# nathancunn/ParticleMDI.jl

Measured on AMD Instinct MI355X. Metric: Gibbs iters/sec (and obs·particles/sec) at 1/2/4/8 GPUs vs CPU ref, higher is better.
Workload: dtype f64

## Files before the change

### particlemdi.jl_amd/csrc/pmdi_sweep2_body.h

```cpp
#pragma once
#include "pmdi_arith.h"
#include "pmdi_internal.h"

#ifndef PM2_LANE_API_PROVIDED
#define PM2_DEV __device__ __forceinline__
#define PM2_COLD __device__ __noinline__
#define PM2_HD inline __host__ __device__
extern __shared__ __attribute__((aligned(16))) unsigned char pm2_smem_[];
#define PM2_SMEM (pm2_smem_)
#define PM2_TID() ((int)threadIdx.x)
#define PM2_BID() ((int)blockIdx.x)
#define PM2_BALLOT(p) __ballot(p)
#define PM2_SHFL64(v, src) pm2_shfl64((v), (src))
#define PM2_WAVE_BARRIER() do { __builtin_amdgcn_fence(__ATOMIC_ACQ_REL, "wavefront"); __builtin_amdgcn_wave_barrier(); } while (0)
#define PM2_BARRIER() __syncthreads()
#define PM2_LDS_BARRIER() asm volatile("s_waitcnt lgkmcnt(0)\n\ts_barrier" ::: "memory")
#define PM2_UNI(x) __builtin_amdgcn_readfirstlane(x)
#define PM2_CLOCK() ((long long)clock64())
#define PM2_WALLCLOCK() ((long long)wall_clock64())
#if defined(__HIP_DEVICE_COMPILE__)
#define PM2_G(T, p) ((__attribute__((address_space(1))) T *)(p))
#define PM2_CONST __attribute__((address_space(4)))
#ifdef PM2_NO_LAUNDER
#define PM2_LAUNDER(ptr_, T) do { } while (0)
// ... 112 lines not shown
#define PHD(i_) PHXW(15)
#define PHR(i_) do { } while (0)
#define PHC(i_) PHXW(i_)
#else
#define PHD(i_) PHX(i_)
#define PHR(i_) do { } while (0)
#define PHC(i_) do { } while (0)
#endif
#else
#define PHD(i_) do { } while (0)
#define PHR(i_) do { } while (0)
#define PHC(i_) do { } while (0)
#endif

typedef unsigned long long u64;
typedef unsigned short u16;
typedef unsigned char u8;

constexpr int NWMAX = 8;
#ifndef PM2_NS
#define PM2_NS 8
#endif
constexpr int NS = PM2_NS;
constexpr int XR = 4;
#ifndef PM2_XCAP
#define PM2_XCAP 24
#endif
constexpr int XCAP = PM2_XCAP;
constexpr int NR = (NS > 2 * XR) ? NS : 2 * XR;
constexpr int CLSMAX = 32;
PM2_HD constexpr int class_slot_bits(int K, int PPL, int NW) { return (K == 4 && PPL == 4 && NW == 4) ? 4 : 5; }
PM2_HD constexpr int class_slots_max(int K, int PPL, int NW) { return 1 << class_slot_bits(K, PPL, NW); }
PM2_HD constexpr bool cdf_rows_in_arena(int NW) { return NW > 4; }
constexpr int KCAPMAX = 256;
constexpr int RI_CLSMIN = 64, RI_NEWSLOT = 96, RI_CLSVAL = 128;
constexpr int RI_WCNT = 160;
constexpr int RD_MAX = 0, RD_MIN = NWMAX, RD_SA = 2 * NWMAX, RD_SQ = 3 * NWMAX;
constexpr int KMAX2 = 4;
constexpr int NONE8 = 0xFF;
constexpr unsigned INFU = 0xFFFFFFFFu;
constexpr int PMDI_S2_REQUEUE = 1;

enum { DS_MAXID = 0, DS_NCLS, DS_NCOL, DS_NDX, DS_ND, DS_NS0, DS_NX, DS_NNEED, DS_NCLONE, DS_NFLAG, DS_FOLLOW, DS_DIRTY, DS_NEEDMASK, DS_CHANGED, DS_NDLOW, DS_HALT, DS_COUNT = 16 };
enum { SC_FAIL = 0, SC_RES, SC_PSTAR, SC_NLEAF, SC_NPROG, SC_JS, SC_TMP0, SC_TMP1, SC_TMP2, SC_TMP3, SC_COUNT = 16 };

typedef S2Layout Layout;

PM2_HD void make_layout(int K, int N, int P, int Dmax, int cols_l, int idcap, int cls, int cdfl, Layout &L)
{
    const int CLS = cls;
    const int kcap = (CLS * N < KCAPMAX) ? CLS * N : KCAPMAX;
    if (cdfl > cls) cdfl = cls;
    L.cls = cls; L.kcap = kcap; L.cdfl = cdfl;
    int o = 0;
    auto take = [&](int bytes) { const int at = o; o = (o + bytes + 15) & ~15; return at; };
    const int Dp = (Dmax + 1) & ~1;
    L.Dp = Dp; L.cols_l = cols_l; L.idcap = idcap;
    L.red = take(128 * 8);
    L.sc = take(SC_COUNT * 4);
    L.stat = take(8 * 8);
    L.wk = take(KMAX2 * 8 * 8);
    L.ph = take(16 * 8);
    L.leaf_i1 = 0; L.leaf_n = 0; L.leaf_prog = 0;
    L.leaf_tot = take(64 * 8); L.leaf_carry = take(64 * 8);
    L.xfl = take(KMAX2 * 64);
    L.tr_tb = 0;
    L.tr_cdf = 128 * 8;
    L.tr_stride = L.tr_cdf + cdfl * (N + 2) * 8;
    if (L.tr_stride < NR * Dp * 8) L.tr_stride = NR * Dp * 8;
    L.tr_stride = (L.tr_stride + 15) & ~15;
    L.rs_jtab = P * 8; L.rs_raw = P * 10; L.rs_anc = P * 12; L.rs_hist = P * 14;
    const int rs = P * 14 + idcap * 4 + 64;
    int trb = K * L.tr_stride;
    if (trb < rs) trb = rs;
    L.tr_bytes = trb;
    L.tr = take(trb);
    const int b0 = o;
// ... 82 lines not shown
    PM2_DEV double *lp() const { return lds<double>(base + lay->lp); }
    PM2_DEV double lp_get(int j) const { if (j < NS + XCAP) return lp()[j]; return PM2_G(const double, ar.lpx())[j - NS - XCAP]; }
    PM2_DEV void lp_set(int j, double x) const { if (j < NS + XCAP) lp()[j] = x; else PM2_G(double, ar.lpx())[j - NS - XCAP] = x; }
    PM2_DEV int xid_get(int e) const { if (e < XCAP) return lds<int>(base + lay->xid)[e]; return PM2_G(const int, ar.xidx())[e - XCAP]; }
    PM2_DEV void xid_set(int e, int id) const { if (e < XCAP) lds<int>(base + lay->xid)[e] = id; else PM2_G(int, ar.xidx())[e - XCAP] = id; }
};

PM2_DEV int popc_below64(const u64 *bm, int p)
{
    int n = 0;
    const int w = p >> 6;
    for (int i = 0; i < w; ++i) n += pm2_popc64(bm[i]);
    return n + pm2_popc64(bm[w] & ((1ull << (p & 63)) - 1ull));
}

template <class Tp, int NN>
struct RegArr {
    Tp head;
    RegArr<Tp, NN - 1> tail;
    PM2_DEV Tp operator[](int i) const { return i == 0 ? head : tail[i - 1]; }
    PM2_DEV void set(int i, Tp x) { head = (i == 0) ? x : head; tail.set(i - 1, x); }
};
template <class Tp>
struct RegArr<Tp, 1> {
    Tp head;
    PM2_DEV Tp operator[](int) const { return head; }
    PM2_DEV void set(int i, Tp x) { head = (i == 0) ? x : head; }
};

template <class Ds> PM2_DEV int ds_levels(const Ds &d) { return d.L; }

template <int K, int PPL, int NW, bool GO> struct Sweep2;
template <int K, int PPL, int NW, bool GO> PM2_COLD void hand_over_cold(Sweep2<K, PPL, NW, GO> s, long long pos, int fcode, long long t_start);

template <int K, int PPL, int NW, bool GO>
struct Sweep2 {
    static constexpr int T = 64 * NW;
    static_assert(NW >= K && NW <= NWMAX, "one owner wave per dataset");
    RegArr<double, PPL> lw;
    static constexpr int NCP = (PPL + 1) / 2;
    RegArr<unsigned, K * NCP> colp;
    static constexpr bool CDFA = cdf_rows_in_arena(NW);
    PM2_DEV double cdf_get(const DV &v, int r, int j) const { if (!CDFA || r < v.cdfl) return v.cdf_row_l(r)[j]; return PM2_G(const double, v.ar.cdfg())[(size_t)r * (N + 2) + j]; }
    PM2_DEV void cdf_set(const DV &v, int r, int j, double x) const { if (!CDFA || r < v.cdfl) v.cdf_row_l(r)[j] = x; else PM2_G(double, v.ar.cdfg())[(size_t)r * (N + 2) + j] = x; }
    static constexpr int CSB = class_slot_bits(K, PPL, NW);
    static constexpr bool ONEWORD = CSB * K * PPL <= 64;
    static constexpr int NCSW = ONEWORD ? 1 : K;
    template <bool Wide, class Dummy = void> struct CslWord { typedef unsigned type; };
    template <class Dummy> struct CslWord<true, Dummy> { typedef u64 type; };
    typedef typename CslWord<(ONEWORD || CSB * PPL > 32)>::type csl_t;
    RegArr<csl_t, NCSW> cslp;
    static_assert(CSB * PPL <= 64, "class slots of a lane's particles of one dataset must fit one 64-bit word");
    RegArr<double, NS> c_mu, c_lam;
#ifdef PM2_DETAIL_TIMERS
    long long phd_last;
    int phd_cur;
#endif
    double pend_g;
    int pend_slot;
    const PM2_CONST SweepArgs *ap;
    int tid, lane, wave, chain;
    int N, P;
    unsigned long long seed;
    unsigned iter;
    long long n, n1;

// ... 992 lines not shown
        const int nb = P >> 6;
        double *lv = car;
        if (wave == 0) {
            if (tid == 0) lds<double>(L.red)[121] = w[0];
            for (int h = 1; (nb >> h) >= 2; ++h) {
                const int cnt = nb >> h, off = nb - (nb >> (h - 1)), offp = (h >= 2) ? nb - (nb >> (h - 2)) : 0;
                if (lane < cnt) {
                    double val;
                    if (h == 1) val = (lane == 0) ? tot[1] : tot[2 * lane] + tot[2 * lane + 1];
                    else val = lv[offp + 2 * lane] + lv[offp + 2 * lane + 1];
                    lv[off + lane] = val;
                }
                PM2_WAVE_BARRIER();
            }
        }
        PM2_BARRIER();
        double carry = lds<double>(L.red)[121];
        if (blk >= 2) {
            const int j = 32 - __builtin_clz((unsigned)blk);
            carry = carry + lv[nb - (nb >> (j - 2))];
            for (int h = j - 2; h >= 0; --h)
                if ((blk >> h) & 1) {
                    const int g = (blk >> h) - 1;
                    carry = carry + (h == 0 ? tot[g] : lv[nb - (nb >> (h - 1)) + g]);
                }
        }
#pragma unroll
        for (int u = 0; u < PPL; ++u) {
            const int p = tid * PPL + u;
            c[u] = (p == 0) ? w[u] : carry + sl[u];
        }
    }

    PM2_DEV void resample(long long pos, double mx)
    {
        PHR(0);
        double w[PPL];
#pragma unroll
        for (int u = 0; u < PPL; ++u) w[u] = exp(lw[u] - mx);
        const double u01 = pmdi_arith::uniform01(seed, iter, (unsigned)pos, 0, 0, SITE_RESAMPLE_U);
        const double usl = pmdi_arith::uniform01(seed, iter, (unsigned)pos, 0, 0, SITE_RESAMPLE_SLOT);
        double c[PPL];
        PHR(1);
        cumsum_pairwise(w, c);
        PHR(2);
        double *utab = lds<double>(L.tr);
        u16 *jtab = lds<u16>(L.tr + L.rs_jtab), *raw = lds<u16>(L.tr + L.rs_raw), *anc = lds<u16>(L.tr + L.rs_anc);
        double *red = lds<double>(L.red);
        if (tid == T - 1) red[0] = c[PPL - 1];
        {
            const double h = 1.0 / (double)P;
            const int j = tid * PPL;
            double u = u01 / (double)P;
            int done = 0;
            while (done < j) {
                int e;
                (void)frexp(u, &e);
                const double B = ldexp(1.0, e);
                const double xx = (B - u) * (double)P;
                double m = floor(xx);
                if (m == xx) m -= 1.0;
                if (m > (double)(j - done)) m = (double)(j - done);
                if (m >= 1.0) { u = u + m * h; done += (int)m; }
                if (done < j) { u = u + h; done += 1; }
            }
#pragma unroll
// ... 9 lines not shown
                int J = (int)((q - utab[0]) * (double)P) + 1;
                if (J < 0) J = 0;
                if (J > P) J = P;
                while (J < P && q >= utab[J]) ++J;
                while (J > 0 && !(q >= utab[J - 1])) --J;
                jtab[tid * PPL + uu] = (u16)J;
            }
        }
        PM2_BARRIER();
        PHR(4);
        {
            int lo = 0;
#pragma unroll
            for (int uu = 0; uu < PPL; ++uu) {
                const int j = tid * PPL + uu;
                if (uu == 0 || !((int)jtab[lo] > j)) {
                    int hi = P - 1;
                    while (lo < hi) { const int mid = (lo + hi) >> 1; if ((int)jtab[mid] > j) hi = mid; else lo = mid + 1; }
                }
                raw[j] = (u16)lo;
            }
        }
        int js = (int)(usl * (double)P);
        if (js >= P) js = P - 1;
        PM2_BARRIER();
        PHR(5);
#pragma unroll
        for (int uu = 0; uu < PPL; ++uu) {
            const int p = tid * PPL + uu;
            anc[p] = (p == 0) ? (u16)0 : (p <= js ? raw[p - 1] : raw[p]);
            lw.set(uu, 1.0);
        }
        PM2_BARRIER();
        u16 *scol = lds<u16>(L.tr), *mult = lds<u16>(L.tr + P * 2), *cmap = lds<u16>(L.tr + P * 4);
        u8 *scsl = lds<u8>(L.tr + P * 6);
        int *hist = lds<int>(L.tr + L.rs_hist);
#pragma nounroll
        for (int k = 0; k < K; ++k) {
            const DV v = view(k);
            int *dsc = v.dsc();
            const int ncol_old = dsc[DS_NCOL], oldmax = dsc[DS_MAXID], ncls_old = dsc[DS_NCLS];
            PHR(6);
            int ck[PPL], rk[PPL];
            col_get(k, ck);
#pragma unroll
            for (int uu = 0; uu < PPL; ++uu) rk[uu] = csl_get(k, uu);
#pragma unroll
            for (int uu = 0; uu < PPL; ++uu) { const int p = tid * PPL + uu; scol[p] = (u16)ck[uu]; scsl[p] = (u8)rk[uu]; }
            for (int e = tid; e < ncol_old; e += T) mult[e] = 0;
            for (int e = tid; e <= oldmax && e < v.idcap; e += T) hist[e] = 0;
            if (tid < CLSMAX) lds<int>(L.red)[RI_CLSMIN + tid] = 0x7fffffff;
            if (tid == 0) sc()[SC_TMP0] = 0;
            PM2_BARRIER();
#pragma unroll
            for (int uu = 0; uu < PPL; ++uu) {
                const int p = tid * PPL + uu;
                const int an = anc[p];
                ck[uu] = scol[an]; rk[uu] = scsl[an];
            }
            PHR(7);
#pragma unroll
            for (int uu = 0; uu < PPL; ++uu) {
                const int cl = ck[uu], r = rk[uu];
                bool start = true;
                if (uu > 0) start = cl != ck[uu - 1] || r != rk[uu - 1];
                int cnt = 1;
// ... 54 lines not shown
                const bool live = occ != 0;
                const u64 bal = PM2_BALLOT(live);
                if (lane == 0) lds<int>(L.red)[RI_WCNT + wave] = pm2_popc64(bal);
                PM2_BARRIER();
                int basew = newmax, tot = 0;
                for (int w_ = 0; w_ < T / 64; ++w_) { const int cnt = lds<int>(L.red)[RI_WCNT + w_]; if (w_ < wave) basew += cnt; tot += cnt; }
                if (id <= oldmax) v.tgt_set(id, live ? basew + pm2_popc64(bal & ((1ull << lane) - 1ull)) + 1 : 0);
                newmax += tot;
                PM2_BARRIER();
            }
            PHR(11);
            for (int b = 0; b < oldmax; b += T) {
                const int id = 1 + b + tid;
                int nid = 0, occ = 0, cnv = 0;
                if (id <= oldmax) {
                    nid = v.tgt_get(id);
                    occ = (id < v.idcap) ? hist[id] : PM2_G(int, v.ar.ncop())[id];
                    cnv = v.cn_get(id);
                    if (id >= v.idcap) PM2_G(int, v.ar.ncop())[id] = 0;
                }
                {
                    const u64 mvb = PM2_BALLOT(nid != 0 && nid != id);
                    if (lane == 0 && mvb) pm2_atomic_add(&sc()[SC_TMP0], pm2_popc64(mvb));
                }
                PM2_BARRIER();
                if (id <= oldmax) {
                    if (nid) { v.counts_set(nid, occ); v.cn_set(nid, cnv); }
                    if (id > newmax) v.counts_set(id, 0);
                }
                PM2_BARRIER();
            }
            PHR(12);
            if (sc()[SC_TMP0] != 0) {
                const int D = ap->ds[k].D;
                if ((GO || v.kind == K_GAUSSIAN)) {
                    auto sb = PM2_G(double, v.ar.sb());
                    const long long nitems = (long long)oldmax * D;
                    for (long long b = 0; b < nitems; b += T) {
                        const long long it = b + tid;
                        const int id = 1 + (int)(it / D), q = (int)(it - (long long)(id - 1) * D);
                        const int nid = (it < nitems) ? v.tgt_get(id) : 0;
                        const bool mv = nid != 0 && nid != id;
                        double sg = 0.0, bt = 0.0;
                        if (mv) { sg = sb[((size_t)id * D + q) * 2]; bt = sb[((size_t)id * D + q) * 2 + 1]; }
                        PM2_BARRIER();
                        if (mv) { sb[((size_t)nid * D + q) * 2] = sg; sb[((size_t)nid * D + q) * 2 + 1] = bt; }
                    }
                } else if ((!GO && v.kind == K_CATEGORICAL)) {
                    auto cn_ = PM2_G(int, v.ar.cnt());
                    const int W = D * v.Lc;
                    const long long nitems = (long long)oldmax * W;
                    for (long long b = 0; b < nitems; b += T) {
                        const long long it = b + tid;
                        const int id = 1 + (int)(it / W), q = (int)(it - (long long)(id - 1) * W);
                        const int nid = (it < nitems) ? v.tgt_get(id) : 0;
                        const bool mv = nid != 0 && nid != id;
                        int c_ = 0;
                        if (mv) c_ = cn_[(size_t)id * W + q];
                        PM2_BARRIER();
                        if (mv) cn_[(size_t)nid * W + q] = c_;
                    }
                } else {
                    auto nb_ = PM2_G(long long, v.ar.nbs());
                    const long long nitems = (long long)oldmax * D;
                    for (long long b = 0; b < nitems; b += T) {
                        const long long it = b + tid;
                        const int id = 1 + (int)(it / D), q = (int)(it - (long long)(id - 1) * D);
                        const int nid = (it < nitems) ? v.tgt_get(id) : 0;
                        const bool mv = nid != 0 && nid != id;
                        long long S_ = 0;
                        if (mv) S_ = nb_[(size_t)id * D + q];
                        PM2_BARRIER();
                        if (mv) nb_[(size_t)nid * D + q] = S_;
                    }
                }
            }
            PM2_BARRIER();
            PHR(13);
            if (wave == k) {
                int *slot_id = lds<int>(v.base + L.slot_id);
                int olds = 0, news = 0;
                if (lane < NS) { olds = slot_id[lane]; news = olds ? v.tgt_get(olds) : 0; }
                PM2_WAVE_BARRIER();
                if (lane < NS && olds) v.slot_set(olds, NONE8);
                PM2_WAVE_BARRIER();
                if (lane < NS) { slot_id[lane] = news; if (news) v.slot_set(news, lane); }
            }
            {
                const int cpr = (2 * T) / N;
                for (int c0 = 0; c0 < ncol_old; c0 += cpr) {
                    int nv[2], dc[2], dn[2];
#pragma unroll
                    for (int h = 0; h < 2; ++h) {
                        const int idx = h * T + tid;
                        const int cc = c0 + idx / N, nn = idx - (idx / N) * N;
                        nv[h] = 0; dc[h] = -1; dn[h] = nn;
                        if (idx < cpr * N && cc < ncol_old && mult[cc] != 0) { nv[h] = v.tgt_get(v.tab_get(cc, nn)); dc[h] = cmap[cc]; }
                    }
                    PM2_BARRIER();
#pragma unroll
                    for (int h = 0; h < 2; ++h) if (dc[h] >= 0) v.tab_set(dc[h], dn[h], nv[h]);
                    PM2_BARRIER();
                }
            }
#pragma unroll
            for (int uu = 0; uu < PPL; ++uu) ck[uu] = cmap[ck[uu]];
            {
// ... 75 lines not shown
        PH2(1);

        double xnext = 0.0;
        int ns0_next = 0;
        int i_next = order[n1 - 1];
        int i_next2 = (n1 < n) ? order[n1] : 0;
        if (owner) {
            xnext = obs_x(wave, i_next);
            ns0_next = PM2_G(const int, a.s_in)[((size_t)chain * K + wave) * n + i_next];
        }
        pend_slot = -1; pend_g = 0.0;
        int failed = 0, handed = 0;
        long long pos_handed = 0;
        for (long long pos = n1 - 1; pos < n; ++pos) {
            PM2_LAUNDER(ap, SweepArgs);
            PM2_FRESH_VGPR(tid); PM2_FRESH_VGPR(lane);
            const double x = xnext;
            const int ns0_cur = ns0_next;
            const int i_cur = i_next;
            if (pos + 1 < n) {
                i_next = i_next2;
                if (owner) {
                    xnext = obs_x(wave, i_next);
                    ns0_next = PM2_G(const int, a.s_in)[((size_t)chain * K + wave) * n + i_next];
                }
                if (pos + 2 < n) i_next2 = order[pos + 2];
            }
            PH2(1);
            if (owner) phase_a(wave, x, ns0_cur, pos);
            PH2(2);
            PM2_BARRIER();
            PH2(3);
            if (sc()[SC_FAIL]) { failed = sc()[SC_FAIL]; break; }
            unsigned nsp[PPL];
#pragma unroll
            for (int u = 0; u < PPL; ++u) nsp[u] = 0;
#pragma nounroll
            for (int k = 0; k < K; ++k) {
                const DV v = view(k);
                const int ns0 = v.dsc()[DS_NS0];
                PHD(5);
                int cl_[PPL], r_[PPL], c_[PPL];
                RegArr<int, PPL> nsv;
                double inc_[PPL];
                bool draw_any = false;
#pragma unroll
                for (int u = 0; u < PPL; ++u) {
                    const int p = tid * PPL + u;
                    r_[u] = csl_get(k, u);
                    cl_[u] = (int)((colp[k * NCP + (u >> 1)] >> ((u & 1) * 16)) & 0xffffu);
                    const int hot = (int)cdf_get(v, r_[u], N + 1);
                    inc_[u] = cdf_get(v, r_[u], N);
                    const int ns = (p == 0) ? ns0 : hot;
                    nsv.set(u, ns);
                    draw_any |= ns < 0;
                }
                PHD(6);
                if (PM2_BALLOT(draw_any)) {
#pragma nounroll
                    for (int u = 0; u < PPL; ++u) {
                        if (nsv[u] < 0) {
                            const int p = tid * PPL + u;
                            const int rr = csl_get(k, u);
                            const double u01 = pmdi_arith::uniform01(seed, iter, (unsigned)pos, (unsigned)k, (unsigned)p, SITE_DRAW);
                            int ns = 0, t = 0;
                            if (!CDFA || rr < v.cdfl) {
                                const double *row = v.cdf_row_l(rr);
                                for (; t + 4 <= N - 1; t += 4) {
                                    const double a0 = row[t], a1 = row[t + 1], a2 = row[t + 2], a3 = row[t + 3];
                                    ns += ((a0 > u01) ? 0 : 1) + ((a1 > u01) ? 0 : 1) + ((a2 > u01) ? 0 : 1) + ((a3 > u01) ? 0 : 1);
                                }
                                for (; t < N - 1; ++t) ns += (row[t] > u01) ? 0 : 1;
                            } else {
                                auto row = PM2_G(const double, v.ar.cdfg()) + (size_t)rr * (N + 2);
                                for (; t < N - 1; ++t) ns += (row[t] > u01) ? 0 : 1;
                            }
                            nsv.set(u, ns);
                        }
                    }
                }
                PHD(7);
                unsigned packed = 0;
#pragma unroll
                for (int u = 0; u < PPL; ++u) {
                    const int ns = nsv[u];
                    lw.set(u, lw[u] + inc_[u]);
                    c_[u] = v.tab_get(cl_[u], ns);
                    nsp[u] |= (unsigned)ns << (8 * k);
                    packed |= (unsigned)ns << (8 * (u & 3));
                    if ((u & 3) == 3 || u == PPL - 1) {
                        u8 *ss = v.ar.sstar() + (size_t)pos * P + (size_t)tid * PPL + (u & ~3);
                        if (PPL >= 4) *PM2_G(unsigned, ss) = packed;
                        else if (PPL == 2) *PM2_G(u16, ss) = (u16)packed;
                        else *PM2_G(u8, ss) = (u8)packed;
                        packed = 0;
                    }
                }
                PHD(8);
                {
                    int keyu[PPL];
#pragma unroll
                    for (int u = 0; u < PPL; ++u) keyu[u] = (r_[u] * P + cl_[u]) * N + nsv[u];
                    bool allsame = true;
#pragma unroll
                    for (int u = 1; u < PPL; ++u) allsame = allsame && keyu[u] == keyu[0];
                    if (PM2_BALLOT(!allsame) == 0) {
                        census(v, true, PPL, r_[0], cl_[0], nsv[0], c_[0], tid * PPL);
                    } else {
#pragma unroll
                        for (int u = 0; u < PPL; ++u) {
                            bool dup = false;
                            int mult = 0;
#pragma unroll
                            for (int u2 = 0; u2 < PPL; ++u2) {
                                const bool same = keyu[u2] == keyu[u];
                                if (u2 < u) dup |= same;
                                if (u2 >= u) mult += same ? 1 : 0;
                            }
                            census(v, !dup, mult, r_[u], cl_[u], nsv[u], c_[u], tid * PPL + u);
                        }
                    }
                }
            }
            PHD(9);
            if (K > 1) {
#pragma unroll
                for (int u = 0; u < PPL; ++u) {
                    int pr = 0;
                    double wv_ = lw[u];
#pragma unroll
                    for (int k1 = 0; k1 < K - 1; ++k1)
#pragma unroll
                        for (int k2 = k1 + 1; k2 < K; ++k2) {
                            wv_ += (((nsp[u] >> (8 * k1)) & 0xffu) == ((nsp[u] >> (8 * k2)) & 0xffu)) ? logphi[pr] : 0.0;
                            ++pr;
                        }
                    lw.set(u, wv_);
                }
            }
            double *red = lds<double>(L.red);
            {
                double mx = lw[0], mn = lw[0];
#pragma unroll
                for (int u = 1; u < PPL; ++u) { mx = (lw[u] > mx) ? lw[u] : mx; mn = (lw[u] < mn) ? lw[u] : mn; }
                mx = wave_max_d(mx); mn = wave_min_d(mn);
                if (lane == 0) { red[RD_MAX + wave] = mx; red[RD_MIN + wave] = mn; }
            }
            PH2(4);
            PM2_BARRIER();
            PH2(5);
            double mx = red[RD_MAX], mn = red[RD_MIN];
            for (int w_ = 1; w_ < NW; ++w_) { mx = (red[RD_MAX + w_] > mx) ? red[RD_MAX + w_] : mx; mn = (red[RD_MIN + w_] < mn) ? red[RD_MIN + w_] : mn; }
            PHD(10);
            const bool lw_flat = mx == mn;
// ... 215 lines not shown
        PM2_BARRIER();
        const int pstar = sc()[SC_PSTAR];
        for (long long pp = tid; pp < n; pp += T) {
            const int i = order[pp];
            for (int k = 0; k < K; ++k) {
                int val;
                if (pp < n1 - 1) val = PM2_G(const int, a.s_in)[((size_t)chain * K + k) * n + i];
                else val = PM2_G(const u8, view(k).ar.sstar())[(size_t)pp * P + pstar];
                PM2_G(int, a.s_out)[((size_t)chain * K + k) * n + i] = val;
            }
        }
        if (a.lw_out)
#pragma unroll
            for (int u = 0; u < PPL; ++u) PM2_G(double, a.lw_out)[(size_t)chain * P + tid * PPL + u] = lw[u];
#pragma nounroll
        for (int k = 0; k < K; ++k) export_dataset(k);
        if (tid == 0) {
            auto st = PM2_G(long long, a.stats) + (size_t)chain * 8;
            const long long *s = stat();
            PM2_G(int, a.pstar)[chain] = pstar;
            st[ST_NOPS] = s[0]; st[ST_NRESAMPLE] = s[1]; st[ST_NCLONES] = s[2]; st[ST_MAXID] = s[3]; st[ST_SUMCLASSES] = s[4];
            st[5] = s[5]; st[6] = 0; st[7] = 0;
            if (!a.err_keep) PM2_G(int, a.err)[chain] = 0;
            if (a.requeue) PM2_G(int, a.requeue)[chain] = 0;
            if (a.swept_by) PM2_G(int, a.swept_by)[chain] = 1;
            PM2_G(long long, a.cost)[chain] = PM2_CLOCK() - t_start;
        }
        if (a.work && tid < K * 8) PM2_G(long long, a.work)[((size_t)chain * PMDI_KMAX_I) * 8 + tid] = lds<long long>(L.wk)[tid];
    }
#undef CLS
#undef L
};

template <int K, int PPL, int NW, bool GO> PM2_COLD void hand_over_cold(Sweep2<K, PPL, NW, GO> s, long long pos, int fcode, long long t_start)
{
    s.hand_over(pos, fcode, t_start);
}

}
```

Before: 886.5.

## Fuse per-dataset resample compaction into one cross-dataset pass with fewer barriers

Adds a fused resample path that handles the ancestor gather, multiplicity histograms, renumbering, moving sufficient statistics and remapping tables for all K datasets together. Work is split into segments, one wave-aligned segment per dataset, so the block-wide barriers are paid once per phase instead of once per dataset. The path is used only when the combined scratch fits in LDS and the ids fit the id capacity; otherwise the old per-dataset loop runs. That loop also now batches the statistic moves four rows per barrier. The fused path is placed in a noinline cold function to limit register pressure, at the cost of call overhead and a lot of new, complex code.

```diff
diff --git a/particlemdi.jl_amd/csrc/pmdi_sweep2_body.h b/particlemdi.jl_amd/csrc/pmdi_sweep2_body.h
--- a/particlemdi.jl_amd/csrc/pmdi_sweep2_body.h
+++ b/particlemdi.jl_amd/csrc/pmdi_sweep2_body.h
@@ -173,12 +173,14 @@
 constexpr int RI_WCNT = 160;
 constexpr int RD_MAX = 0, RD_MIN = NWMAX, RD_SA = 2 * NWMAX, RD_SQ = 3 * NWMAX;
 constexpr int KMAX2 = 4;
+constexpr int MVR = 4;
+constexpr int WK_FUSED = 7;
 constexpr int NONE8 = 0xFF;
 constexpr unsigned INFU = 0xFFFFFFFFu;
 constexpr int PMDI_S2_REQUEUE = 1;
 
 enum { DS_MAXID = 0, DS_NCLS, DS_NCOL, DS_NDX, DS_ND, DS_NS0, DS_NX, DS_NNEED, DS_NCLONE, DS_NFLAG, DS_FOLLOW, DS_DIRTY, DS_NEEDMASK, DS_CHANGED, DS_NDLOW, DS_HALT, DS_COUNT = 16 };
-enum { SC_FAIL = 0, SC_RES, SC_PSTAR, SC_NLEAF, SC_NPROG, SC_JS, SC_TMP0, SC_TMP1, SC_TMP2, SC_TMP3, SC_COUNT = 16 };
+enum { SC_FAIL = 0, SC_RES, SC_PSTAR, SC_NLEAF, SC_NPROG, SC_JS, SC_TMP0, SC_TMP1, SC_TMP2, SC_TMP3, SC_MV0 , SC_COUNT = 16 };
 
 typedef S2Layout Layout;
 
@@ -327,6 +329,8 @@
 
 template <int K, int PPL, int NW, bool GO> struct Sweep2;
 template <int K, int PPL, int NW, bool GO> PM2_COLD void hand_over_cold(Sweep2<K, PPL, NW, GO> s, long long pos, int fcode, long long t_start);
+template <int K, int PPL, int NW, bool GO> struct FusedLane;
+template <int K, int PPL, int NW, bool GO> PM2_COLD FusedLane<K, PPL, NW, GO> resample_fused_cold(const SweepArgs *ap, int chain, FusedLane<K, PPL, NW, GO> fl);
 
 template <int K, int PPL, int NW, bool GO>
 struct Sweep2 {
@@ -1385,6 +1389,414 @@
         }
     }
 
+    struct Mv { double a, b; long long c; };
+    PM2_DEV int mv_words(const DV &v, int k) const { return ((!GO && v.kind == K_CATEGORICAL)) ? ap->ds[k].D * v.Lc : ap->ds[k].D; }
+    PM2_DEV Mv mv_load(const DV &v, int W, int id, int q) const
+    {
+        Mv m;
+        m.a = 0.0; m.b = 0.0; m.c = 0;
+        if ((GO || v.kind == K_GAUSSIAN)) {
+            auto sb = PM2_G(const double, v.ar.sb());
+            m.a = sb[((size_t)id * W + q) * 2]; m.b = sb[((size_t)id * W + q) * 2 + 1];
+        } else if ((!GO && v.kind == K_CATEGORICAL)) {
+            m.c = PM2_G(const int, v.ar.cnt())[(size_t)id * W + q];
+        } else {
+            m.c = PM2_G(const long long, v.ar.nbs())[(size_t)id * W + q];
+        }
+        return m;
+    }
+    PM2_DEV void mv_store(const DV &v, int W, int nid, int q, const Mv &m) const
+    {
+        if ((GO || v.kind == K_GAUSSIAN)) {
+            auto sb = PM2_G(double, v.ar.sb());
+            sb[((size_t)nid * W + q) * 2] = m.a; sb[((size_t)nid * W + q) * 2 + 1] = m.b;
+        } else if ((!GO && v.kind == K_CATEGORICAL)) {
+            PM2_G(int, v.ar.cnt())[(size_t)nid * W + q] = (int)m.c;
+        } else {
+            PM2_G(long long, v.ar.nbs())[(size_t)nid * W + q] = m.c;
+        }
+    }
+    PM2_DEV int seg_find(const int (&sz)[K], int cs, int &s0) const
+    {
+        int k = -1, st = 0;
+        s0 = 0;
+#pragma unroll
+        for (int kk = 0; kk < K; ++kk) {
+            const int psz = (sz[kk] + 63) & ~63;
+            if (cs >= st && cs < st + psz) { k = kk; s0 = st; }
+            st += psz;
+        }
+        return k;
+    }
+    PM2_DEV int seg_total(const int (&sz)[K]) const
+    {
+        int st = 0;
+#pragma unroll
+        for (int kk = 0; kk < K; ++kk) st += (sz[kk] + 63) & ~63;
+        return st;
+    }
+    PM2_DEV int pick(const int (&a)[K], int k) const
+    {
+        int r = a[0];
+#pragma unroll
+        for (int kk = 1; kk < K; ++kk) r = (kk == k) ? a[kk] : r;
+        return r;
+    }
+
+    PM2_DEV void resample_fused()
+    {
+        int nco[K], om[K], ncl[K];
+#pragma unroll
+        for (int k = 0; k < K; ++k) {
+            const int *dsc = lds<int>(L.ds0 + k * L.ds_stride + L.dsc);
+            nco[k] = PM2_UNI(dsc[DS_NCOL]); om[k] = PM2_UNI(dsc[DS_MAXID]); ncl[k] = PM2_UNI(dsc[DS_NCLS]);
+        }
+        const u16 *anc = lds<u16>(L.tr + L.rs_anc);
+        int *redi = lds<int>(L.red);
+        PHR(6);
+        {
+            u16 *scol = lds<u16>(L.tr);
+            u8 *scsl = lds<u8>(L.tr + K * P * 2);
+#pragma unroll
+            for (int k = 0; k < K; ++k) {
+                int ck[PPL];
+                col_get(k, ck);
+#pragma unroll
+                for (int uu = 0; uu < PPL; ++uu) { const int p = tid * PPL + uu; scol[k * P + p] = (u16)ck[uu]; scsl[k * P + p] = (u8)csl_get(k, uu); }
+            }
+            PM2_BARRIER();
+            int an[PPL];
+#pragma unroll
+            for (int uu = 0; uu < PPL; ++uu) an[uu] = anc[tid * PPL + uu];
+#pragma unroll
+            for (int k = 0; k < K; ++k) {
+                int ck[PPL];
+#pragma unroll
+                for (int uu = 0; uu < PPL; ++uu) { ck[uu] = scol[k * P + an[uu]]; csl_put(k, uu, (int)scsl[k * P + an[uu]]); }
+                col_put(k, ck);
+            }
+            PM2_BARRIER();
+        }
+        int ho[K], co[K], mo[K];
+        int nints = 0, nu16 = 0;
+#pragma unroll
+        for (int k = 0; k < K; ++k) {
+            ho[k] = nints; nints += om[k] + 1;
+            co[k] = nints; nints += 3 * ncl[k];
+            mo[k] = nu16; nu16 += 2 * ((nco[k] + 1) & ~1);
+        }
+        int *ti = lds<int>(L.tr);
+        u16 *tu = lds<u16>(L.tr + nints * 4);
+        for (int e = tid; e < nints + nu16 / 2; e += T) {
+            bool cm = false;
+#pragma unroll
+            for (int k = 0; k < K; ++k) cm = cm || (e >= co[k] && e < co[k] + ncl[k]);
+            ti[e] = cm ? 0x7fffffff : 0;
+        }
+        if (tid < K) sc()[SC_MV0 + tid] = 0;
+        PM2_BARRIER();
+        PHR(7);
+#pragma nounroll
+        for (int k = 0; k < K; ++k) {
+            int ck[PPL], rk[PPL];
+            col_get(k, ck);
+#pragma unroll
+            for (int uu = 0; uu < PPL; ++uu) rk[uu] = csl_get(k, uu);
+            u16 *mult = tu + pick(mo, k);
+            int *clsmin = ti + pick(co, k);
+#pragma unroll
+            for (int uu = 0; uu < PPL; ++uu) {
+                const int cl = ck[uu], r = rk[uu];
+                bool start = true;
+                if (uu > 0) start = cl != ck[uu - 1] || r != rk[uu - 1];
+                int cnt = 1;
+                {
+                    bool go = true;
+#pragma unroll
+                    for (int u2 = uu + 1; u2 < PPL; ++u2) { go = go && ck[u2] == cl && rk[u2] == r; cnt += go ? 1 : 0; }
+                }
+                const u64 act = PM2_BALLOT(start);
+                if (act) {
+                    const int l0 = pm2_ffs64(act) - 1;
+                    const int key = cl * CLSMAX + r;
+                    const int key0 = readlane_i(key, l0);
+                    const bool uni = PM2_BALLOT(start && key == key0) == act;
+                    int tot = cnt;
+                    if (uni) {
+                        tot = 0;
+#pragma unroll
+                        for (int c_ = 1; c_ <= PPL; ++c_) tot += c_ * pm2_popc64(PM2_BALLOT(start && cnt == c_));
+                    }
+                    if (uni ? (lane == l0) : start) {
+                        pm2_atomic_add((unsigned *)mult + (cl >> 1), (unsigned)tot << ((cl & 1) * 16));
+                        pm2_atomic_min(&clsmin[r], tid * PPL + uu);
+                    }
+                }
+            }
+        }
+        PM2_BARRIER();
+        PHR(9);
+        {
+            int sz[K];
+#pragma unroll
+            for (int k = 0; k < K; ++k) sz[k] = nco[k] * N;
+            const int tot = seg_total(sz);
+            for (int b = 0; b < tot; b += T) {
+                int s0;
+                const int cs = b + wave * 64;
+                int k = seg_find(sz, cs, s0);
+                if (k >= 0) {
+                    k = PM2_UNI(k);
+                    const int i = cs - s0 + lane;
+                    if (i < pick(sz, k)) {
+                        const int cc = i / N;
+                        const int m = (tu + pick(mo, k))[cc];
+                        if (m) { const DV v = view(k); pm2_atomic_add(ti + pick(ho, k) + v.tab_get(cc, i - cc * N), m); }
+                    }
+                }
+            }
+        }
+        PHR(8);
+        int ncn[K], nmx[K];
+        int par = 0;
+#pragma unroll
+        for (int k = 0; k < K; ++k) { ncn[k] = 0; nmx[k] = 0; }
+        {
+            const int tot = seg_total(nco);
+            for (int b = 0; b < tot; b += T, par ^= 1) {
+                int s0;
+                const int cs = b + wave * 64;
+                const int k = seg_find(nco, cs, s0);
+                const int i = cs - s0 + lane;
+                u16 *mult = tu + pick(mo, k);
+                bool live = false;
+                if (k >= 0 && i < pick(nco, k)) live = mult[i] != 0;
+                const u64 bal = PM2_BALLOT(live);
+                if (lane == 0) redi[RI_WCNT + par * NWMAX + wave] = pm2_popc64(bal);
+                PM2_BARRIER();
+                int base = pick(ncn, k);
+#pragma unroll
+                for (int w_ = 0; w_ < NW; ++w_) {
+                    int s1;
+                    const int kw = seg_find(nco, b + w_ * 64, s1);
+                    const int cnt = redi[RI_WCNT + par * NWMAX + w_];
+                    if (w_ < wave && kw == k) base += cnt;
+#pragma unroll
+                    for (int kk = 0; kk < K; ++kk) ncn[kk] += (kw == kk) ? cnt : 0;
+                }
+                if (live) (mult + ((pick(nco, k) + 1) & ~1))[i] = (u16)(base + pm2_popc64(bal & ((1ull << lane) - 1ull)));
+            }
+            PM2_BARRIER();
+        }
+        PHR(10);
+        {
+            const int tot = seg_total(om);
+            for (int b = 0; b < tot; b += T, par ^= 1) {
+                int s0;
+                const int cs = b + wave * 64;
+                const int k = seg_find(om, cs, s0);
+                const int id = 1 + cs - s0 + lane;
+                const bool in = k >= 0 && id <= pick(om, k);
+                bool live = false;
+                if (in) live = (ti + pick(ho, k))[id] != 0;
+                const u64 bal = PM2_BALLOT(live);
+                if (lane == 0) redi[RI_WCNT + par * NWMAX + wave] = pm2_popc64(bal);
+                PM2_BARRIER();
+                int base = pick(nmx, k);
+#pragma unroll
+                for (int w_ = 0; w_ < NW; ++w_) {
+                    int s1;
+                    const int kw = seg_find(om, b + w_ * 64, s1);
+                    const int cnt = redi[RI_WCNT + par * NWMAX + w_];
+                    if (w_ < wave && kw == k) base += cnt;
+#pragma unroll
+                    for (int kk = 0; kk < K; ++kk) nmx[kk] += (kw == kk) ? cnt : 0;
+                }
+                if (in) lds<int>(L.ds0 + k * L.ds_stride + L.tgt)[id] = live ? base + pm2_popc64(bal & ((1ull << lane) - 1ull)) + 1 : 0;
+            }
+            PM2_BARRIER();
+        }
+        PHR(11);
+        {
+            const int tot = seg_total(om);
+            for (int b = 0; b < tot; b += T) {
+                int s0;
+                const int cs = b + wave * 64;
+                const int k = seg_find(om, cs, s0);
+                const int id = 1 + cs - s0 + lane;
+                const bool in = k >= 0 && id <= pick(om, k);
+                const int dbase = L.ds0 + k * L.ds_stride;
+                int nid = 0, occ = 0, cnv = 0;
+                if (in) { nid = lds<int>(dbase + L.tgt)[id]; occ = (ti + pick(ho, k))[id]; cnv = lds<int>(dbase + L.cn)[id]; }
+                {
+                    const u64 mvb = PM2_BALLOT(nid != 0 && nid != id);
+                    if (lane == 0 && mvb) pm2_atomic_add(&sc()[SC_MV0 + k], pm2_popc64(mvb));
+                }
+                PM2_BARRIER();
+                if (in) {
+                    if (nid) { lds<int>(dbase + L.counts)[nid] = occ; lds<int>(dbase + L.cn)[nid] = cnv; }
+                    if (id > pick(nmx, k)) lds<int>(dbase + L.counts)[id] = 0;
+                }
+            }
+        }
+        PHR(12);
+        {
+            int sz[K], any = 0;
+#pragma unroll
+            for (int k = 0; k < K; ++k) {
+                const int moved = PM2_UNI(sc()[SC_MV0 + k]);
+                sz[k] = 0;
+                if (moved) { const DV v = view(k); sz[k] = om[k] * mv_words(v, k); }
+                any |= moved;
+            }
+            const int tot = any ? seg_total(sz) : 0;
+            for (int b = 0; b < tot; b += MVR * T) {
+                int nidr[MVR];
+                Mv mv[MVR];
+#pragma unroll
+                for (int r = 0; r < MVR; ++r) {
+                    int s0;
+                    const int cs = b + r * T + wave * 64;
+                    int k = seg_find(sz, cs, s0);
+                    nidr[r] = 0; mv[r].a = 0.0; mv[r].b = 0.0; mv[r].c = 0;
+                    if (k >= 0) {
+                        k = PM2_UNI(k);
+                        const int i = cs - s0 + lane;
+                        if (i < pick(sz, k)) {
+                            const DV v = view(k);
+                            const int W = mv_words(v, k);
+                            const int id = 1 + i / W, q = i - (id - 1) * W;
+                            const int nid = lds<int>(v.base + L.tgt)[id];
+                            if (nid != 0 && nid != id) { nidr[r] = nid; mv[r] = mv_load(v, W, id, q); }
+                        }
+                    }
+                }
+                PM2_BARRIER();
+#pragma unroll
+                for (int r = 0; r < MVR; ++r) {
+                    int s0;
+                    const int cs = b + r * T + wave * 64;
+                    int k = seg_find(sz, cs, s0);
+                    if (k >= 0) {
+                        k = PM2_UNI(k);
+                        if (nidr[r]) {
+                            const DV v = view(k);
+                            const int W = mv_words(v, k);
+                            const int i = cs - s0 + lane;
+                            const int id = 1 + i / W, q = i - (id - 1) * W;
+                            mv_store(v, W, nidr[r], q, mv[r]);
+                        }
+                    }
+                }
+            }
+        }
+        PHR(13);
+        if (wave < K) {
+            const DV v = view(wave);
+            int *slot_id = lds<int>(v.base + L.slot_id);
+            int olds = 0, news = 0;
+            if (lane < NS) { olds = slot_id[lane]; news = olds ? v.tgt_get(olds) : 0; }
+            PM2_WAVE_BARRIER();
+            if (lane < NS && olds) v.slot_set(olds, NONE8);
+            PM2_WAVE_BARRIER();
+            if (lane < NS) { slot_id[lane] = news; if (news) v.slot_set(news, lane); }
+        }
+        {
+            int sz[K];
+#pragma unroll
+            for (int k = 0; k < K; ++k) sz[k] = nco[k] * N;
+            const int tot = seg_total(sz);
+            for (int b = 0; b < tot; b += 2 * T) {
+                int nv[2], dc[2];
+#pragma unroll
+                for (int h = 0; h < 2; ++h) {
+                    int s0;
+                    const int cs = b + h * T + wave * 64;
+                    int k = seg_find(sz, cs, s0);
+                    nv[h] = 0; dc[h] = -1;
+                    if (k >= 0) {
+                        k = PM2_UNI(k);
+                        const int i = cs - s0 + lane;
+                        if (i < pick(sz, k)) {
+                            const int cc = i / N;
+                            const u16 *mult = tu + pick(mo, k);
+                            if (mult[cc] != 0) {
+                                const DV v = view(k);
+                                nv[h] = lds<int>(v.base + L.tgt)[v.tab_get(cc, i - cc * N)];
+                                dc[h] = (mult + ((pick(nco, k) + 1) & ~1))[cc];
+                            }
+                        }
+                    }
+                }
+                PM2_BARRIER();
+#pragma unroll
+                for (int h = 0; h < 2; ++h) {
+                    int s0;
+                    const int cs = b + h * T + wave * 64;
+                    int k = seg_find(sz, cs, s0);
+                    if (k >= 0) {
+                        k = PM2_UNI(k);
+                        if (dc[h] >= 0) {
+                            const DV v = view(k);
+                            const int i = cs - s0 + lane;
+                            v.tab_set(dc[h], i - (i / N) * N, nv[h]);
+                        }
+                    }
+                }
+            }
+        }
+        {
+            int k = -1, r = 0, st = 0;
+#pragma unroll
+            for (int kk = 0; kk < K; ++kk) {
+                if (tid >= st && tid < st + ncl[kk]) { k = kk; r = tid - st; }
+                st += ncl[kk];
+            }
+            if (k >= 0) {
+                const int nc = pick(ncl, k);
+                int *cm = ti + pick(co, k);
+                const int mine = cm[r];
+                int s = 0;
+                for (int r2 = 0; r2 < nc; ++r2) if (cm[r2] < mine) ++s;
+                cm[nc + r] = s;
+                cm[2 * nc + r] = lds<int>(L.ds0 + k * L.ds_stride + L.clsval)[r];
+            }
+        }
+        PM2_BARRIER();
+#pragma nounroll
+        for (int k = 0; k < K; ++k) {
+            const int dbase = L.ds0 + k * L.ds_stride;
+            const int nc = pick(ncl, k);
+            const int *cm = ti + pick(co, k);
+            const u16 *cmap = tu + pick(mo, k) + ((pick(nco, k) + 1) & ~1);
+            int ck[PPL];
+            col_get(k, ck);
+#pragma unroll
+            for (int uu = 0; uu < PPL; ++uu) {
+                const int p = tid * PPL + uu;
+                const int r = csl_get(k, uu);
+                const int ns_ = cm[nc + r];
+                ck[uu] = cmap[ck[uu]];
+                if (cm[r] == p) { lds<int>(dbase + L.clsval)[ns_] = cm[2 * nc + r]; lds<int>(dbase + L.clslead)[ns_] = p; lds<int>(dbase + L.leadcol)[ns_] = ck[uu]; }
+                csl_put(k, uu, ns_);
+            }
+            col_put(k, ck);
+        }
+        if (tid < K) {
+            const int k = tid;
+            const int nc = pick(ncl, k);
+            const int *cm = ti + pick(co, k);
+            int nc2 = 0;
+            for (int r = 0; r < nc; ++r) nc2 += (cm[r] != 0x7fffffff) ? 1 : 0;
+            int *dsc = lds<int>(L.ds0 + k * L.ds_stride + L.dsc);
+            const int moved = sc()[SC_MV0 + k];
+            dsc[DS_NCLS] = nc2; dsc[DS_NCOL] = pick(ncn, k); dsc[DS_MAXID] = pick(nmx, k); dsc[DS_DIRTY] = 1;
+            long long *w_ = wk(k);
+            w_[WK_COLS] += pick(nco, k); w_[WK_MOVED] += moved; w_[WK_MOVE_EVENTS] += moved ? 1 : 0; w_[WK_FUSED] += 1;
+        }
+        PM2_BARRIER();
+    }
+
     PM2_DEV void resample(long long pos, double mx)
     {
         PHR(0);
@@ -1460,6 +1872,32 @@
             lw.set(uu, 1.0);
         }
         PM2_BARRIER();
+        {
+            int nco[K], om[K], ncl[K];
+            int bytes = 0;
+            bool fits = true;
+#pragma unroll
+            for (int k = 0; k < K; ++k) {
+                const int *dsc = lds<int>(L.ds0 + k * L.ds_stride + L.dsc);
+                nco[k] = PM2_UNI(dsc[DS_NCOL]); om[k] = PM2_UNI(dsc[DS_MAXID]); ncl[k] = PM2_UNI(dsc[DS_NCLS]);
+                bytes += 4 * (om[k] + 1 + 3 * ncl[k]) + 4 * ((nco[k] + 1) & ~1);
+                fits = fits && om[k] < L.idcap;
+            }
+            if (fits && bytes <= L.rs_anc) {
+                FusedLane<K, PPL, NW, GO> fl;
+                fl.colp = colp; fl.cslp = cslp;
+#ifdef PM2_DETAIL_TIMERS
+                fl.phd_last = phd_last; fl.phd_cur = phd_cur;
+#endif
+                fl = resample_fused_cold<K, PPL, NW, GO>((const SweepArgs *)ap, chain, fl);
+                colp = fl.colp; cslp = fl.cslp;
+#ifdef PM2_DETAIL_TIMERS
+                phd_last = fl.phd_last; phd_cur = fl.phd_cur;
+#endif
+                PHR(15);
+                return;
+            }
+        }
         u16 *scol = lds<u16>(L.tr), *mult = lds<u16>(L.tr + P * 2), *cmap = lds<u16>(L.tr + P * 4);
         u8 *scsl = lds<u8>(L.tr + P * 6);
         int *hist = lds<int>(L.tr + L.rs_hist);
@@ -1580,47 +2018,29 @@
             }
             PHR(12);
             if (sc()[SC_TMP0] != 0) {
-                const int D = ap->ds[k].D;
-                if ((GO || v.kind == K_GAUSSIAN)) {
-                    auto sb = PM2_G(double, v.ar.sb());
-                    const long long nitems = (long long)oldmax * D;
-                    for (long long b = 0; b < nitems; b += T) {
-                        const long long it = b + tid;
-                        const int id = 1 + (int)(it / D), q = (int)(it - (long long)(id - 1) * D);
-                        const int nid = (it < nitems) ? v.tgt_get(id) : 0;
-                        const bool mv = nid != 0 && nid != id;
-                        double sg = 0.0, bt = 0.0;
-                        if (mv) { sg = sb[((size_t)id * D + q) * 2]; bt = sb[((size_t)id * D + q) * 2 + 1]; }
-                        PM2_BARRIER();
-                        if (mv) { sb[((size_t)nid * D + q) * 2] = sg; sb[((size_t)nid * D + q) * 2 + 1] = bt; }
-                    }
-                } else if ((!GO && v.kind == K_CATEGORICAL)) {
-                    auto cn_ = PM2_G(int, v.ar.cnt());
-                    const int W = D * v.Lc;
-                    const long long nitems = (long long)oldmax * W;
-                    for (long long b = 0; b < nitems; b += T) {
-                        const long long it = b + tid;
-                        const int id = 1 + (int)(it / W), q = (int)(it - (long long)(id - 1) * W);
-                        const int nid = (it < nitems) ? v.tgt_get(id) : 0;
-                        const bool mv = nid != 0 && nid != id;
-                        int c_ = 0;
-                        if (mv) c_ = cn_[(size_t)id * W + q];
-                        PM2_BARRIER();
-                        if (mv) cn_[(size_t)nid * W + q] = c_;
-                    }
-                } else {
-                    auto nb_ = PM2_G(long long, v.ar.nbs());
-                    const long long nitems = (long long)oldmax * D;
-                    for (long long b = 0; b < nitems; b += T) {
-                        const long long it = b + tid;
-                        const int id = 1 + (int)(it / D), q = (int)(it - (long long)(id - 1) * D);
-                        const int nid = (it < nitems) ? v.tgt_get(id) : 0;
-                        const bool mv = nid != 0 && nid != id;
-                        long long S_ = 0;
-                        if (mv) S_ = nb_[(size_t)id * D + q];
-                        PM2_BARRIER();
-                        if (mv) nb_[(size_t)nid * D + q] = S_;
-                    }
+                const int W = mv_words(v, k);
+                const long long nitems = (long long)oldmax * W;
+                for (long long b = 0; b < nitems; b += (long long)MVR * T) {
+                    int nidr[MVR];
+                    Mv mv[MVR];
+#pragma unroll
+                    for (int r = 0; r < MVR; ++r) {
+                        const long long it = b + (long long)r * T + tid;
+                        nidr[r] = 0; mv[r].a = 0.0; mv[r].b = 0.0; mv[r].c = 0;
+                        if (it < nitems) {
+                            const int id = 1 + (int)(it / W), q = (int)(it - (long long)(id - 1) * W);
+                            const int nid = v.tgt_get(id);
+                            if (nid != 0 && nid != id) { nidr[r] = nid; mv[r] = mv_load(v, W, id, q); }
+                        }
+                    }
+                    PM2_BARRIER();
+#pragma unroll
+                    for (int r = 0; r < MVR; ++r)
+                        if (nidr[r]) {
+                            const long long it = b + (long long)r * T + tid;
+                            const int id = 1 + (int)(it / W), q = (int)(it - (long long)(id - 1) * W);
+                            mv_store(v, W, nidr[r], q, mv[r]);
+                        }
                 }
             }
             PM2_BARRIER();
@@ -2131,6 +2551,32 @@
 #undef L
 };
 
+template <int K, int PPL, int NW, bool GO> struct FusedLane {
+    decltype(Sweep2<K, PPL, NW, GO>::colp) colp;
+    decltype(Sweep2<K, PPL, NW, GO>::cslp) cslp;
+#ifdef PM2_DETAIL_TIMERS
+    long long phd_last;
+    int phd_cur;
+#endif
+};
+template <int K, int PPL, int NW, bool GO> PM2_COLD FusedLane<K, PPL, NW, GO> resample_fused_cold(const SweepArgs *ap, int chain, FusedLane<K, PPL, NW, GO> fl)
+{
+    Sweep2<K, PPL, NW, GO> s;
+    s.ap = (const PM2_CONST SweepArgs *)ap; s.chain = chain;
+    s.tid = PM2_TID(); s.lane = s.tid & 63; s.wave = s.tid >> 6;
+    s.N = s.ap->N; s.P = s.ap->P;
+    s.colp = fl.colp; s.cslp = fl.cslp;
+#ifdef PM2_DETAIL_TIMERS
+    s.phd_last = fl.phd_last; s.phd_cur = fl.phd_cur;
+#endif
+    s.resample_fused();
+    fl.colp = s.colp; fl.cslp = s.cslp;
+#ifdef PM2_DETAIL_TIMERS
+    fl.phd_last = s.phd_last; fl.phd_cur = s.phd_cur;
+#endif
+    return fl;
+}
+
 template <int K, int PPL, int NW, bool GO> PM2_COLD void hand_over_cold(Sweep2<K, PPL, NW, GO> s, long long pos, int fcode, long long t_start)
 {
     s.hand_over(pos, fcode, t_start);
```

Result: slower. 852.3 (-3.8%).

## Batch particle CDF loads and table lookups across pairs of datasets

Applied to the files above, without the earlier changes.

Restructures the per-dataset particle loop to process datasets in groups of PD (default 2). The hot/inc CDF reads and the class-table lookups for every dataset in a group are issued up front, so their memory latency overlaps before the census work runs. Sampled states are now kept packed in nsp, with 0xff used as the marker for 'needs draw'. This raises register pressure and adds per-dataset ballot checks in exchange for more memory-level parallelism.

```diff
diff --git a/particlemdi.jl_amd/csrc/pmdi_sweep2_body.h b/particlemdi.jl_amd/csrc/pmdi_sweep2_body.h
--- a/particlemdi.jl_amd/csrc/pmdi_sweep2_body.h
+++ b/particlemdi.jl_amd/csrc/pmdi_sweep2_body.h
@@ -168,6 +168,10 @@
 PM2_HD constexpr int class_slot_bits(int K, int PPL, int NW) { return (K == 4 && PPL == 4 && NW == 4) ? 4 : 5; }
 PM2_HD constexpr int class_slots_max(int K, int PPL, int NW) { return 1 << class_slot_bits(K, PPL, NW); }
 PM2_HD constexpr bool cdf_rows_in_arena(int NW) { return NW > 4; }
+#ifndef PM2_PP_DEPTH
+#define PM2_PP_DEPTH 2
+#endif
+PM2_HD constexpr int particle_depth(int K, int , int ) { return K < PM2_PP_DEPTH ? K : PM2_PP_DEPTH; }
 constexpr int KCAPMAX = 256;
 constexpr int RI_CLSMIN = 64, RI_NEWSLOT = 96, RI_CLSVAL = 128;
 constexpr int RI_WCNT = 160;
@@ -1762,94 +1766,148 @@
             PM2_BARRIER();
             PH2(3);
             if (sc()[SC_FAIL]) { failed = sc()[SC_FAIL]; break; }
-            unsigned nsp[PPL];
-#pragma unroll
-            for (int u = 0; u < PPL; ++u) nsp[u] = 0;
+            RegArr<unsigned, PPL> nsp;
+#pragma unroll
+            for (int u = 0; u < PPL; ++u) nsp.set(u, 0u);
+            constexpr int PD = particle_depth(K, PPL, NW);
 #pragma nounroll
-            for (int k = 0; k < K; ++k) {
-                const DV v = view(k);
-                const int ns0 = v.dsc()[DS_NS0];
+            for (int k0 = 0; k0 < K; k0 += PD) {
                 PHD(5);
-                int cl_[PPL], r_[PPL], c_[PPL];
-                RegArr<int, PPL> nsv;
-                double inc_[PPL];
                 bool draw_any = false;
-#pragma unroll
-                for (int u = 0; u < PPL; ++u) {
-                    const int p = tid * PPL + u;
-                    r_[u] = csl_get(k, u);
-                    cl_[u] = (int)((colp[k * NCP + (u >> 1)] >> ((u & 1) * 16)) & 0xffffu);
-                    const int hot = (int)cdf_get(v, r_[u], N + 1);
-                    inc_[u] = cdf_get(v, r_[u], N);
-                    const int ns = (p == 0) ? ns0 : hot;
-                    nsv.set(u, ns);
-                    draw_any |= ns < 0;
+                {
+                    int hot_[PD][PPL];
+                    double inc_[PD][PPL];
+#pragma unroll
+                    for (int j = 0; j < PD; ++j) {
+#pragma unroll
+                        for (int u = 0; u < PPL; ++u) { hot_[j][u] = 0; inc_[j][u] = 0.0; }
+                        const int k = k0 + j;
+                        if (k < K) {
+                            const DV v = view(k);
+#pragma unroll
+                            for (int u = 0; u < PPL; ++u) {
+                                const int r = csl_get(k, u);
+                                hot_[j][u] = (int)cdf_get(v, r, N + 1);
+                                inc_[j][u] = cdf_get(v, r, N);
+                            }
+                        }
+                    }
+#pragma unroll
+                    for (int j = 0; j < PD; ++j) {
+                        const int k = k0 + j;
+                        if (k < K) {
+                            const int ns0 = view(k).dsc()[DS_NS0];
+#pragma unroll
+                            for (int u = 0; u < PPL; ++u) {
+                                const int p = tid * PPL + u;
+                                const int ns = (p == 0) ? ns0 : hot_[j][u];
+                                lw.set(u, lw[u] + inc_[j][u]);
+                                nsp.set(u, nsp[u] | (((unsigned)ns & 0xffu) << (8 * k)));
+                                draw_any |= ns < 0;
+                            }
+                        }
+                    }
                 }
                 PHD(6);
                 if (PM2_BALLOT(draw_any)) {
 #pragma nounroll
+                    for (int k = k0; k < k0 + PD && k < K; ++k) {
+                        bool mine = false;
+#pragma unroll
+                        for (int u = 0; u < PPL; ++u) mine |= ((nsp[u] >> (8 * k)) & 0xffu) == 0xffu;
+                        if (!PM2_BALLOT(mine)) continue;
+                        const DV v = view(k);
+#pragma nounroll
+                        for (int u = 0; u < PPL; ++u) {
+                            if (((nsp[u] >> (8 * k)) & 0xffu) == 0xffu) {
+                                const int p = tid * PPL + u;
+                                const int rr = csl_get(k, u);
+                                const double u01 = pmdi_arith::uniform01(seed, iter, (unsigned)pos, (unsigned)k, (unsigned)p, SITE_DRAW);
+                                int ns = 0, t = 0;
+                                if (!CDFA || rr < v.cdfl) {
+                                    const double *row = v.cdf_row_l(rr);
+                                    for (; t + 4 <= N - 1; t += 4) {
+                                        const double a0 = row[t], a1 = row[t + 1], a2 = row[t + 2], a3 = row[t + 3];
+                                        ns += ((a0 > u01) ? 0 : 1) + ((a1 > u01) ? 0 : 1) + ((a2 > u01) ? 0 : 1) + ((a3 > u01) ? 0 : 1);
+                                    }
+                                    for (; t < N - 1; ++t) ns += (row[t] > u01) ? 0 : 1;
+                                } else {
+                                    auto row = PM2_G(const double, v.ar.cdfg()) + (size_t)rr * (N + 2);
+                                    for (; t < N - 1; ++t) ns += (row[t] > u01) ? 0 : 1;
+                                }
+                                nsp.set(u, nsp[u] ^ ((0xffu ^ (unsigned)ns) << (8 * k)));
+                            }
+                        }
+                    }
+                }
+                PHD(7);
+                int c_[PD][PPL];
+#pragma unroll
+                for (int j = 0; j < PD; ++j) {
+#pragma unroll
+                    for (int u = 0; u < PPL; ++u) c_[j][u] = 0;
+                    const int k = k0 + j;
+                    if (k < K) {
+                        const DV v = view(k);
+                        int ck[PPL];
+                        col_get(k, ck);
+#pragma unroll
+                        for (int u = 0; u < PPL; ++u) c_[j][u] = v.tab_get(ck[u], (int)((nsp[u] >> (8 * k)) & 0xffu));
+                    }
+                }
+#pragma nounroll
+                for (int j = 0; j < PD; ++j) {
+                    const int k = k0 + j;
+                    if (k >= K) break;
+                    const DV v = view(k);
+                    int cl_[PPL], r_[PPL], ns_[PPL], cj[PPL];
+                    col_get(k, cl_);
+#pragma unroll
                     for (int u = 0; u < PPL; ++u) {
-                        if (nsv[u] < 0) {
-                            const int p = tid * PPL + u;
-                            const int rr = csl_get(k, u);
-                            const double u01 = pmdi_arith::uniform01(seed, iter, (unsigned)pos, (unsigned)k, (unsigned)p, SITE_DRAW);
-                            int ns = 0, t = 0;
-                            if (!CDFA || rr < v.cdfl) {
-                                const double *row = v.cdf_row_l(rr);
-                                for (; t + 4 <= N - 1; t += 4) {
-                                    const double a0 = row[t], a1 = row[t + 1], a2 = row[t + 2], a3 = row[t + 3];
-                                    ns += ((a0 > u01) ? 0 : 1) + ((a1 > u01) ? 0 : 1) + ((a2 > u01) ? 0 : 1) + ((a3 > u01) ? 0 : 1);
+                        r_[u] = csl_get(k, u);
+                        ns_[u] = (int)((nsp[u] >> (8 * k)) & 0xffu);
+                        cj[u] = c_[0][u];
+#pragma unroll
+                        for (int j2 = 1; j2 < PD; ++j2) cj[u] = (j2 == j) ? c_[j2][u] : cj[u];
+                    }
+                    unsigned packed = 0;
+#pragma unroll
+                    for (int u = 0; u < PPL; ++u) {
+                        packed |= (unsigned)ns_[u] << (8 * (u & 3));
+                        if ((u & 3) == 3 || u == PPL - 1) {
+                            u8 *ss = v.ar.sstar() + (size_t)pos * P + (size_t)tid * PPL + (u & ~3);
+                            if (PPL >= 4) *PM2_G(unsigned, ss) = packed;
+                            else if (PPL == 2) *PM2_G(u16, ss) = (u16)packed;
+                            else *PM2_G(u8, ss) = (u8)packed;
+                            packed = 0;
+                        }
+                    }
+                    PHD(8);
+                    {
+                        int keyu[PPL];
+#pragma unroll
+                        for (int u = 0; u < PPL; ++u) keyu[u] = (r_[u] * P + cl_[u]) * N + ns_[u];
+                        bool allsame = true;
+#pragma unroll
+                        for (int u = 1; u < PPL; ++u) allsame = allsame && keyu[u] == keyu[0];
+                        if (PM2_BALLOT(!allsame) == 0) {
+                            census(v, true, PPL, r_[0], cl_[0], ns_[0], cj[0], tid * PPL);
+                        } else {
+#pragma unroll
+                            for (int u = 0; u < PPL; ++u) {
+                                bool dup = false;
+                                int mult = 0;
+#pragma unroll
+                                for (int u2 = 0; u2 < PPL; ++u2) {
+                                    const bool same = keyu[u2] == keyu[u];
+                                    if (u2 < u) dup |= same;
+                                    if (u2 >= u) mult += same ? 1 : 0;
                                 }
-                                for (; t < N - 1; ++t) ns += (row[t] > u01) ? 0 : 1;
-                            } else {
-                                auto row = PM2_G(const double, v.ar.cdfg()) + (size_t)rr * (N + 2);
-                                for (; t < N - 1; ++t) ns += (row[t] > u01) ? 0 : 1;
+                                census(v, !dup, mult, r_[u], cl_[u], ns_[u], cj[u], tid * PPL + u);
                             }
-                            nsv.set(u, ns);
                         }
                     }
-                }
-                PHD(7);
-                unsigned packed = 0;
-#pragma unroll
-                for (int u = 0; u < PPL; ++u) {
-                    const int ns = nsv[u];
-                    lw.set(u, lw[u] + inc_[u]);
-                    c_[u] = v.tab_get(cl_[u], ns);
-                    nsp[u] |= (unsigned)ns << (8 * k);
-                    packed |= (unsigned)ns << (8 * (u & 3));
-                    if ((u & 3) == 3 || u == PPL - 1) {
-                        u8 *ss = v.ar.sstar() + (size_t)pos * P + (size_t)tid * PPL + (u & ~3);
-                        if (PPL >= 4) *PM2_G(unsigned, ss) = packed;
-                        else if (PPL == 2) *PM2_G(u16, ss) = (u16)packed;
-                        else *PM2_G(u8, ss) = (u8)packed;
-                        packed = 0;
-                    }
-                }
-                PHD(8);
-                {
-                    int keyu[PPL];
-#pragma unroll
-                    for (int u = 0; u < PPL; ++u) keyu[u] = (r_[u] * P + cl_[u]) * N + nsv[u];
-                    bool allsame = true;
-#pragma unroll
-                    for (int u = 1; u < PPL; ++u) allsame = allsame && keyu[u] == keyu[0];
-                    if (PM2_BALLOT(!allsame) == 0) {
-                        census(v, true, PPL, r_[0], cl_[0], nsv[0], c_[0], tid * PPL);
-                    } else {
-#pragma unroll
-                        for (int u = 0; u < PPL; ++u) {
-                            bool dup = false;
-                            int mult = 0;
-#pragma unroll
-                            for (int u2 = 0; u2 < PPL; ++u2) {
-                                const bool same = keyu[u2] == keyu[u];
-                                if (u2 < u) dup |= same;
-                                if (u2 >= u) mult += same ? 1 : 0;
-                            }
-                            census(v, !dup, mult, r_[u], cl_[u], nsv[u], c_[u], tid * PPL + u);
-                        }
-                    }
+                    PHD(7);
                 }
             }
             PHD(9);
```

Measured after the change: 886.3 before, 886.1 after. No clear change (-0.0%).
